# mush42/sonata

Measured on NVIDIA H100. Metric: audio-sec/sec, higher is better.
Workload: dtype f32 io; wgmma with split operands (2 x bf16 flow/decoder, 3 x tf32 encoder/predictor), fp32 accumulate

## Files before the change

### include/sonata_b200.h

```cpp
#ifndef SONATA_B200_H
#define SONATA_B200_H

#include <stddef.h>
#include <stdint.h>

#ifdef __cplusplus
extern "C" {
#endif

#define SB200_OK 0
#define SB200_FAILED_TO_LOAD_RESOURCE 17
#define SB200_PHONEMIZATION_ERROR 18
#define SB200_OPERATION_ERROR 19

typedef struct sb200_voice sb200_voice;
typedef struct sb200_job sb200_job;
typedef struct sb200_latent sb200_latent;

typedef struct sb200_error {
    int32_t code;
    char* message;
} sb200_error;

typedef struct sb200_audio {
// ... 77 lines not shown
int32_t sb200_encode_ids(sb200_voice* v, const int64_t* ids, size_t n, sb200_latent** out, sb200_error* err);
int64_t sb200_latent_frames(const sb200_latent* z);
int32_t sb200_decode_chunk(sb200_voice* v, const sb200_latent* z, int64_t frame_lo, int64_t frame_hi,
                           sb200_audio* out, sb200_error* err);
void sb200_latent_free(sb200_latent* z);

int32_t sb200_encode_batch_ids_configs(sb200_voice* v, const int64_t* ids_packed, const size_t* offsets, size_t batch,
                                       const sb200_synth_config* cfgs, sb200_latent** outs, sb200_error* err);
int32_t sb200_encode_batch_ids_durations(sb200_voice* v, const int64_t* ids_packed, const size_t* offsets, size_t batch,
                                         const sb200_synth_config* cfgs, const float* scale_packed,
                                         const int32_t* frames_packed, sb200_latent** outs, sb200_error* err);
int64_t sb200_latent_id_frames(const sb200_latent* z, int32_t* out, size_t capacity);
int32_t sb200_decode_chunks(sb200_voice* v, const sb200_latent* const* zs, const int64_t* lo, const int64_t* hi, size_t n,
                            sb200_audio* outs, sb200_error* err);
int32_t sb200_decode_chunks_i16(sb200_voice* v, const sb200_latent* const* zs, const int64_t* lo, const int64_t* hi,
                                const int64_t* trim_lo_frames, const int64_t* trim_hi_frames, size_t n, int32_t fade,
                                const float* gain, int16_t** outs, size_t* lens, sb200_error* err);

int32_t sb200_job_debug_fetch(sb200_job* job, const char* name, size_t b, float** data, size_t* rows, size_t* cols,
                              sb200_error* err);
void sb200_buffer_free(float* p);
int32_t sb200_job_debug_durations(sb200_job* job, size_t b, int32_t** cum, size_t* n, sb200_error* err);

typedef struct sb200_region_stat {
    char name[32];
    double ms;
    double flops;
    double bytes;
    int32_t launches;
} sb200_region_stat;
int32_t sb200_job_profile(const sb200_job* job, sb200_region_stat* out, int32_t cap);
int32_t sb200_debug_plan(int32_t backend, int64_t rows, int32_t cin, int32_t cout, int32_t k, int32_t dil, int32_t act,
                         int32_t has_res, int32_t accumulate, int32_t* out16);
int32_t sb200_debug_conv_grid_cap(int32_t cap);
int32_t sb200_debug_conv(int32_t device, int32_t backend, const float* x, int32_t rows, int32_t cin, const float* w,
                         const float* bias, int32_t cout, int32_t k, int32_t dil, float in_slope, int32_t act,
                         const float* res, float scale, int32_t accumulate, float* y, int32_t valid_rows,
                         sb200_error* err);
int32_t sb200_debug_conv_ex(int32_t device, int32_t backend, const float* x, int32_t rows, int32_t cin, const float* w,
                            const float* bias, int32_t cout, int32_t k, int32_t dil, float in_slope, int32_t act,
                            const float* res, float scale, const int32_t* seg_end, int32_t gran, int32_t seg_mul,
                            float* y0, int32_t acc0, int32_t split, float* y1, int32_t acc1, sb200_error* err);
int32_t sb200_debug_spline(int32_t device, const float* h29, int32_t ldh, float* z, int32_t rows, int32_t tcol,
                           int32_t valid_rows, sb200_error* err);
int32_t sb200_debug_durations(int32_t device, const float* z, int32_t rows, const int32_t* seg_off, const int32_t* seg_len,
                              int32_t nseg, float m0, float logs0, float length_scale, float* logw, int32_t* cum,
                              int32_t* y_len, sb200_error* err);
uint64_t sb200_launch_count(void);
int32_t sb200_set_backend(sb200_voice* v, int32_t backend);

#ifdef __cplusplus
}
#endif
#endif
```

### sonata_b200/_native.py

```python
from __future__ import annotations

import ctypes as C
import os

_HERE = os.path.dirname(os.path.abspath(__file__))
LIB_PATH = os.environ.get("SB200_LIB") or os.path.join(_HERE, "lib", "libsonata_b200.so")


class sb200_error(C.Structure):
    _fields_ = [("code", C.c_int32), ("message", C.c_void_p)]


class sb200_audio(C.Structure):
    _fields_ = [("data", C.POINTER(C.c_float)), ("len", C.c_size_t), ("inference_ms", C.c_float),
                ("sample_rate", C.c_uint32)]


class sb200_synth_config(C.Structure):
    _fields_ = [("speaker", C.c_int64), ("has_speaker", C.c_int32), ("noise_scale", C.c_float),
                ("length_scale", C.c_float), ("noise_w", C.c_float)]


class sb200_audio_info(C.Structure):
    _fields_ = [("sample_rate", C.c_uint32), ("num_channels", C.c_uint32), ("sample_width", C.c_uint32)]
# ... 50 lines not shown
    "sb200_job_fetch": (C.c_int32, [_P, C.POINTER(sb200_audio), _ERR]),
    "sb200_job_fetch_i16": (C.c_int32, [_P, C.POINTER(C.POINTER(C.c_int16)), C.POINTER(C.c_size_t), _ERR]),
    "sb200_i16_free": (None, [C.POINTER(C.c_int16)]),
    "sb200_job_batch": (C.c_size_t, [_P]),
    "sb200_job_lengths": (C.c_int32, [_P, C.POINTER(C.c_int64), C.POINTER(C.c_int64), C.POINTER(C.c_int64)]),
    "sb200_job_copy_out": (C.c_int32, [_P, C.c_void_p, C.c_size_t, C.c_int32, C.POINTER(C.c_size_t), _ERR]),
    "sb200_host_register": (C.c_int32, [C.c_void_p, C.c_size_t, _ERR]),
    "sb200_host_unregister": (C.c_int32, [C.c_void_p]),
    "sb200_job_free": (None, [_P]),
    "sb200_encode_ids": (C.c_int32, [_P, C.POINTER(C.c_int64), C.c_size_t, C.POINTER(_P), _ERR]),
    "sb200_latent_frames": (C.c_int64, [_P]),
    "sb200_decode_chunk": (C.c_int32, [_P, _P, C.c_int64, C.c_int64, C.POINTER(sb200_audio), _ERR]),
    "sb200_latent_free": (None, [_P]),
    "sb200_encode_batch_ids_configs": (C.c_int32, [_P, C.POINTER(C.c_int64), C.POINTER(C.c_size_t), C.c_size_t,
                                                   C.POINTER(sb200_synth_config), C.POINTER(_P), _ERR]),
    "sb200_encode_batch_ids_durations": (C.c_int32, [_P, C.POINTER(C.c_int64), C.POINTER(C.c_size_t), C.c_size_t,
                                                     C.POINTER(sb200_synth_config), C.POINTER(C.c_float),
                                                     C.POINTER(C.c_int32), C.POINTER(_P), _ERR]),
    "sb200_latent_id_frames": (C.c_int64, [_P, C.POINTER(C.c_int32), C.c_size_t]),
    "sb200_decode_chunks": (C.c_int32, [_P, C.POINTER(_P), C.POINTER(C.c_int64), C.POINTER(C.c_int64), C.c_size_t,
                                        C.POINTER(sb200_audio), _ERR]),
    "sb200_decode_chunks_i16": (C.c_int32, [_P, C.POINTER(_P), C.POINTER(C.c_int64), C.POINTER(C.c_int64),
                                            C.POINTER(C.c_int64), C.POINTER(C.c_int64), C.c_size_t, C.c_int32,
                                            C.POINTER(C.c_float), C.POINTER(C.POINTER(C.c_int16)),
                                            C.POINTER(C.c_size_t), _ERR]),
    "sb200_job_debug_fetch": (C.c_int32, [_P, C.c_char_p, C.c_size_t, C.POINTER(C.POINTER(C.c_float)),
                                          C.POINTER(C.c_size_t), C.POINTER(C.c_size_t), _ERR]),
    "sb200_buffer_free": (None, [C.POINTER(C.c_float)]),
    "sb200_job_debug_durations": (C.c_int32, [_P, C.c_size_t, C.POINTER(C.POINTER(C.c_int32)),
                                              C.POINTER(C.c_size_t), _ERR]),
    "sb200_job_profile": (C.c_int32, [_P, C.POINTER(sb200_region_stat), C.c_int32]),
    "sb200_debug_plan": (C.c_int32, [C.c_int32, C.c_int64, C.c_int32, C.c_int32, C.c_int32, C.c_int32, C.c_int32, C.c_int32,
                                      C.c_int32, C.POINTER(C.c_int32)]),
    "sb200_debug_conv_grid_cap": (C.c_int32, [C.c_int32]),
    "sb200_debug_conv": (C.c_int32, [C.c_int32, C.c_int32, C.POINTER(C.c_float), C.c_int32, C.c_int32,
                                     C.POINTER(C.c_float), C.POINTER(C.c_float), C.c_int32, C.c_int32, C.c_int32,
                                     C.c_float, C.c_int32, C.POINTER(C.c_float), C.c_float, C.c_int32,
                                     C.POINTER(C.c_float), C.c_int32, _ERR]),
    "sb200_debug_conv_ex": (C.c_int32, [C.c_int32, C.c_int32, C.POINTER(C.c_float), C.c_int32, C.c_int32,
                                        C.POINTER(C.c_float), C.POINTER(C.c_float), C.c_int32, C.c_int32, C.c_int32,
                                        C.c_float, C.c_int32, C.POINTER(C.c_float), C.c_float, C.POINTER(C.c_int32),
                                        C.c_int32, C.c_int32, C.POINTER(C.c_float), C.c_int32, C.c_int32,
                                        C.POINTER(C.c_float), C.c_int32, _ERR]),
    "sb200_debug_spline": (C.c_int32, [C.c_int32, C.POINTER(C.c_float), C.c_int32, C.POINTER(C.c_float), C.c_int32,
                                       C.c_int32, C.c_int32, _ERR]),
    "sb200_debug_durations": (C.c_int32, [C.c_int32, C.POINTER(C.c_float), C.c_int32, C.POINTER(C.c_int32),
                                          C.POINTER(C.c_int32), C.c_int32, C.c_float, C.c_float, C.c_float,
                                          C.POINTER(C.c_float), C.POINTER(C.c_int32), C.POINTER(C.c_int32), _ERR]),
    "sb200_launch_count": (C.c_uint64, []),
    "sb200_set_backend": (C.c_int32, [_P, C.c_int32]),
}

_lib = None


def lib() -> C.CDLL:
    global _lib
    if _lib is None:
        if not os.path.exists(LIB_PATH):
            raise ImportError(
                f"{LIB_PATH} is missing: run `python -c 'import __graft_entry__ as g; g.build()'` "
                "(libsonata_b200 has no CPU fallback)")
        l = C.CDLL(LIB_PATH)
        for name, (res, args) in SIGNATURES.items():
            fn = getattr(l, name)
            fn.restype = res
# ... 4 lines not shown
```

### sonata_b200/csrc/capi.cu

```cuda
#include "../../include/sonata_b200.h"
#include "engine.h"
#include "tc_common.cuh"
#include <algorithm>
#include <chrono>
#include <cstring>
#include <deque>

using namespace sb200;

struct sb200_voice { std::shared_ptr<Voice> v; };
struct sb200_job {
    Job* j; std::shared_ptr<Voice> keep;
    ~sb200_job() { delete j; }
};
struct sb200_latent {
    Latent* l; std::shared_ptr<Voice> keep;
    ~sb200_latent() { delete l; }
};

namespace {

struct PinnedBlock { std::atomic<int> refs{0}; float* base = nullptr; size_t bytes = 0; };
std::mutex g_pin_mu;
std::deque<PinnedBlock*> g_pin_free;
// ... 422 lines not shown
        SB_CUDA(cudaSetDevice(j.v->device));
        if (U < 0) {
            SB_CUDA(cudaMemcpy2D(*data, nr * 4, it->second.first + r0, (size_t)j.RX * 4, nr * 4, (size_t)C, cudaMemcpyDeviceToHost));
            *rows = (size_t)C; *cols = nr;
            return;
        }
        SB_CUDA(cudaMemcpy(*data, it->second.first + r0 * C, nr * C * 4, cudaMemcpyDeviceToHost));
        *rows = nr; *cols = (size_t)C;
    });
}
int32_t sb200_job_debug_durations(sb200_job* job, size_t b, int32_t** cum, size_t* n, sb200_error* err) {
    return guarded(err, [&] {
        Job& j = *job->j;
        if (!j.ran) throw Error(19, "job not run");
        const size_t len = (size_t)j.xsegs[b].len;
        *cum = (int32_t*)malloc(len * 4 + 4);
        SB_CUDA(cudaSetDevice(j.v->device));
        SB_CUDA(cudaMemcpy(*cum, j.d_cum + j.xsegs[b].off, len * 4, cudaMemcpyDeviceToHost));
        *n = len;
    });
}
int32_t sb200_job_profile(const sb200_job* job, sb200_region_stat* out, int32_t cap) {
    const Job& j = *job->j;
    int32_t n = 0;
    for (const Region& r : j.regions) {
        if (n >= cap) break;
        memset(&out[n], 0, sizeof(out[n]));
        strncpy(out[n].name, r.name.c_str(), sizeof(out[n].name) - 1);
        out[n].ms = r.ms; out[n].flops = r.flops; out[n].bytes = r.bytes; out[n].launches = r.launches;
        n++;
    }
    return n;
}
int32_t sb200_debug_plan(int32_t backend, int64_t rows, int32_t cin, int32_t cout, int32_t k, int32_t dil, int32_t act,
                         int32_t has_res, int32_t accumulate, int32_t* out16) {
    if (!out16 || cin <= 0 || cout <= 0 || k <= 0 || k > SB_MAX_TAPS || dil <= 0 || rows <= 0) return 19;
    static float anchor[64];
    float* const stand_in = reinterpret_cast<float*>((reinterpret_cast<uintptr_t>(anchor) + 127) & ~(uintptr_t)127);
    ConvArgs p{};
    const int R = (int)((rows + 255) / 256 * 256);
    const int ycols = act == ACT_GATE ? cout / 2 : cout;
    p.x = stand_in; p.ldx = cin; p.rows_in = R; p.cin = cin; p.in_slope = 0.1f;
    p.w = stand_in; p.bias = stand_in; p.ldw = cout; p.cout = cout;
    p.tc_nt = cout <= 128 ? cout : (cout % 128 == 0 ? 128 : (cout % 96 == 0 ? 96 : 0));
    p.wtc = p.tc_nt ? stand_in : nullptr; p.wtf = stand_in;
    p.ntaps = k;
    for (int t = 0; t < k; t++) p.tap_off[t] = (t - (k - 1) / 2) * dil;
    p.min_off = p.tap_off[0]; p.span = (k - 1) * dil;
    p.rows_q = R; p.orow_mul = 1; p.orow_add = 0;
    p.act = act; p.scale = 1.f; p.res = has_res ? stand_in : nullptr; p.ldres = cout;
    p.y0 = stand_in; p.ldy0 = ycols; p.acc0 = accumulate; p.split = cout; p.y1 = stand_in; p.ldy1 = ycols; p.acc1 = accumulate;
    const bool ok = backend == 2 ? conv_tf_plan_info(p, out16) : conv_tc_plan_info(p, out16);
    return ok ? 0 : 19;
}

int32_t sb200_debug_conv_grid_cap(int32_t cap) {
    const int32_t old = g_conv_tc_grid_cap;
    g_conv_tc_grid_cap = cap > 0 ? cap : 0;
    return old;
}

int32_t sb200_debug_conv_ex(int32_t device, int32_t backend, const float* x, int32_t rows, int32_t cin, const float* w,
                            const float* bias, int32_t cout, int32_t k, int32_t dil, float in_slope, int32_t act,
                            const float* res, float scale, const int32_t* seg_end, int32_t gran, int32_t seg_mul,
                            float* y0, int32_t acc0, int32_t split, float* y1, int32_t acc1, sb200_error* err) {
    return guarded(err, [&] {
        if (rows <= 0 || gran <= 0 || seg_mul <= 0 || !seg_end) throw Error(19, "debug conv: bad row map");
        if (split < 0 || split > cout) split = cout;
        if (split < cout && (act == ACT_GATE || !y1)) throw Error(19, "debug conv: a split output needs y1 and no gate");
        SB_CUDA(cudaSetDevice(device));
        Voice tmp; tmp.device = device;
        ConvW cw = debug_make_conv(tmp, w, bias, cout, cin, k, dil);
        const int R = (rows + 255) / 256 * 256;
        const int ycols = act == ACT_GATE ? cout / 2 : cout;
        const int ld0 = std::min(split, ycols), ld1 = cout - split;
        const int ngran = (R + gran - 1) / gran;
        std::vector<int> ends(ngran, 0);
        for (int g = 0; g < ngran && g * gran < rows; g++) ends[g] = seg_end[g];
        float *dx, *dy0 = nullptr, *dy1 = nullptr, *dres = nullptr; int* dend;
        SB_CUDA(cudaMalloc(&dx, (size_t)R * cin * 4)); SB_CUDA(cudaMemset(dx, 0, (size_t)R * cin * 4));
        SB_CUDA(cudaMemcpy(dx, x, (size_t)rows * cin * 4, cudaMemcpyHostToDevice));
        auto upload_y = [&](float*& d, const float* h, int ld) {
            if (ld <= 0) return;
            SB_CUDA(cudaMalloc(&d, (size_t)R * ld * 4)); SB_CUDA(cudaMemset(d, 0, (size_t)R * ld * 4));
            SB_CUDA(cudaMemcpy(d, h, (size_t)rows * ld * 4, cudaMemcpyHostToDevice));
        };
// ... 101 lines not shown
```

### sonata_b200/csrc/common.cuh

```cuda
#pragma once
#include <cuda_runtime.h>
#include <stdint.h>
#include <stdlib.h>
#include <mutex>

#define SB_MAX_TAPS 16

namespace sb200 {

struct RowMap {
    const int* seg_end;
    int gran;
    int seg_mul;
    int rows;
};

__device__ __forceinline__ bool row_valid(const RowMap& m, int q) {
    if (q < 0 || q >= m.rows) return false;
    return q < m.seg_end[q / m.gran] * m.seg_mul;
}

enum ConvAct { ACT_NONE = 0, ACT_RELU = 1, ACT_GATE = 2 };

struct ConvArgs {
// ... 41 lines not shown
    unsigned long long done = 0;
    template <typename F> void run(F&& f) {
        int dev = 0;
        cudaGetDevice(&dev);
        const unsigned long long bit = 1ull << (dev & 63);
        if (__atomic_load_n(&done, __ATOMIC_ACQUIRE) & bit) return;
        std::lock_guard<std::mutex> g(mu);
        if (done & bit) return;
        f();
        __atomic_fetch_or(&done, bit, __ATOMIC_RELEASE);
    }
};

__device__ __forceinline__ void pdl_wait() { asm volatile("griddepcontrol.wait;" ::: "memory"); }
__device__ __forceinline__ void pdl_trigger() { asm volatile("griddepcontrol.launch_dependents;" ::: "memory"); }

template <typename... KArgs, typename... Args>
inline void launch_pdl(void (*kern)(KArgs...), dim3 grid, dim3 block, size_t smem, cudaStream_t st, Args&&... args) {
    static const int allowed = getenv("SB200_NO_PDL") ? 0 : 1;
    cudaLaunchConfig_t cfg{};
    cfg.gridDim = grid; cfg.blockDim = block; cfg.dynamicSmemBytes = smem; cfg.stream = st;
    cudaLaunchAttribute at[1];
    at[0].id = cudaLaunchAttributeProgrammaticStreamSerialization;
    at[0].val.programmaticStreamSerializationAllowed = allowed;
    cfg.attrs = at; cfg.numAttrs = 1;
    cudaLaunchKernelEx(&cfg, kern, KArgs(args)...);
}

#define SB_ENV_ONCE(name) ([]() -> const char* { static const char* v = getenv(name); return v; }())

void launch_conv_simt(const ConvArgs& a, cudaStream_t st);
int conv_simt_bn_for(int cout);
bool conv_tc_supported(const ConvArgs& a);
bool conv_tc_plan_info(const ConvArgs& a, int* out16);
void launch_conv_tc(const ConvArgs& a, cudaStream_t st);
bool try_launch_conv_tc(const ConvArgs& a, cudaStream_t st);
extern int g_conv_tc_grid_cap;
size_t conv_tc_weight_floats(int cin, int cout, int ntaps, int nt);
void conv_tc_build_weights(const float* wt, int ldw, int cin, int cout, int ntaps, int nt, float* out);
bool conv_tf_supported(const ConvArgs& a);
bool conv_tf_plan_info(const ConvArgs& a, int* out16);
void launch_conv_tf(const ConvArgs& a, cudaStream_t st);
bool try_launch_conv_tf(const ConvArgs& a, cudaStream_t st);
size_t conv_tf_weight_floats(int cin, int cout, int ntaps);
void conv_tf_build_weights(const float* wt, int ldw, int cin, int cout, int ntaps, float* out);
bool gemm_tf_supported(const TfGemm& g);
void launch_gemm_tf(const TfGemm& g, cudaStream_t st);
void throw_launch_error(const char* what);

struct SegInfo { int off; int len; };

void launch_embed(const int* ids_rows, const float* emb, float scale, float* x, int rows, int H, cudaStream_t st);
void launch_ln(const float* x, const float* res1, const float* res2, const float* gamma, const float* beta,
               float* out, int C, int act, RowMap map, cudaStream_t st);
void launch_dw_ln_gelu(const float* x, const float* wdw , const float* bdw, int k, int dil,
                       const float* gamma, const float* beta, float* out, int C, RowMap map, cudaStream_t st);
void launch_attn_softmax(float* S, int Tp, const float* qkv, int ldq, const float* relk, const float* relv, int window,
                         float* orel, int ldo, int H, int heads, int RX, const SegInfo* segs, const int* seg_of_gran,
                         int gran, int max_len, cudaStream_t st);
void launch_attention(const float* qkv, int ldq, const float* relk, const float* relv, int window,
                      float* out, int ldo, int H, int heads, const SegInfo* segs, int nseg, int max_len,
                      cudaStream_t st);
size_t attention_smem_bytes(int max_len, int D);
void launch_flow_pre(const float* z, int zcol, const float* w, const float* b, const float* g, float* h,
                     int C, RowMap map, cudaStream_t st);
void launch_spline(const float* h29, int ldh, float* z, int tcol, int bins, float inv_sqrt_filter,
                   RowMap map, cudaStream_t st);
// ... 24 lines not shown
```

### sonata_b200/csrc/conv_tc.cu

```cuda
#include "tc_common.cuh"
#include <algorithm>
#include <stdlib.h>
#include <string.h>

namespace sb200 {

int g_conv_tc_grid_cap = 0;

int wg_num_sms() {
    static int n = 0;
    if (!n) {
        int dev = 0;
        if (cudaGetDevice(&dev) != cudaSuccess || cudaDeviceGetAttribute(&n, cudaDevAttrMultiProcessorCount, dev) != cudaSuccess)
            cudaGetLastError();
        if (n <= 0) n = 132;
    }
    return n;
}

namespace {

using namespace tcx;

struct TcLaunch {
    int nt;
    int wnt;
    int win;
    int ntiles_m, ntiles_n;
    int grid;
    int resident;
    int pairs;
};

constexpr int TC_CONSUMERS = 256;
constexpr int TC_STAGES = 2;
constexpr int TC_BAR_BYTES = 64;

template <int NT> struct TcRoles {
    static constexpr int ctas = NT == 32 ? 2 : 1;
    static constexpr int producers = NT == 32 ? 128 : 256;
    static constexpr int threads = TC_CONSUMERS + producers;
    static constexpr int launch = (65536 / (threads * ctas)) & ~7;
    static constexpr int producer_regs = NT == 32 ? 40 : 32;
    static constexpr int consumer_regs = ((launch * threads - producer_regs * producers) / TC_CONSUMERS) & ~7;
};

template <int NT>
__global__ void __launch_bounds__(TcRoles<NT>::threads, TcRoles<NT>::ctas) conv_tc_kernel(const ConvArgs a, const TcLaunch L) {
    constexpr int NPROD = TcRoles<NT>::producers;
    pdl_trigger();
    extern __shared__ __align__(1024) uint8_t smem_raw[];
    uint8_t* smem = reinterpret_cast<uint8_t*>((reinterpret_cast<uintptr_t>(smem_raw) + 1023) & ~(uintptr_t)1023);
    const int nkb = a.cin / 32, S = TC_STAGES;
    const uint32_t a_buf = (uint32_t)L.win * 128u;
    const uint32_t w_tap = (uint32_t)NT * 128u;
    const uint32_t w_kb = (uint32_t)a.ntaps * w_tap;
    const uint32_t w_bytes = L.resident ? (uint32_t)nkb * w_kb : (uint32_t)S * w_kb;
    const uint32_t A0 = smem_u32(smem), W0 = A0 + S * a_buf;
    const uint32_t FULL = A0 + S * a_buf + w_bytes;
    const uint32_t EMPTY = FULL + 8u * TC_STAGES;
    const uint32_t WRES = EMPTY + 8u * TC_STAGES;
    const int tid = threadIdx.x;
    const int n_tile = (int)blockIdx.x % L.ntiles_n, m_first = (int)blockIdx.x / L.ntiles_n;
    const int m_step = (int)gridDim.x / L.ntiles_n;
    const int nsteps = (L.ntiles_m - m_first + m_step - 1) / m_step * nkb;

    if (tid == 0) {
        for (int s = 0; s < S; s++) {
            mbar_init(FULL + 8u * s, NPROD + (L.resident ? 0 : 1));
            mbar_init(EMPTY + 8u * s, TC_CONSUMERS);
        }
        mbar_init(WRES, 1);
        asm volatile("fence.mbarrier_init.release.cluster;" ::: "memory");
    }
    __syncthreads();

    if (tid >= TC_CONSUMERS) {
        setmaxnreg_dec<TcRoles<NT>::producer_regs>();
        const int ptid = tid - TC_CONSUMERS;
        const int vf = L.wnt / NT;
        const size_t w_image = (size_t)L.wnt * 128u;
        const uint8_t* wsrc = reinterpret_cast<const uint8_t*>(a.wtc) + (size_t)(n_tile / vf) * nkb * a.ntaps * w_image +
                              (size_t)(n_tile % vf) * w_tap;
        auto issue_w = [&](int kb0, int nkb_, uint32_t dst, uint32_t bar) {
            if (ptid == 0) {
                mbar_expect_tx(bar, (uint32_t)nkb_ * w_kb);
                for (int i = 0; i < nkb_ * a.ntaps; i++)
                    bulk_g2s(dst + i * w_tap, wsrc + (size_t)(kb0 * a.ntaps + i) * w_image, w_tap, bar);
            }
        };
        auto issue_a = [&](int j, int s) {
            const int kb = j % nkb, rbase = (m_first + j / nkb * m_step) * 128 + a.min_off;
            for (int idx = ptid; idx < L.win * 8; idx += NPROD) {
                const int gr = rbase + (idx >> 3);
                const bool ok = gr >= 0 && gr < a.rows_in;
                const float* src = ok ? a.x + (size_t)gr * a.ldx + kb * 32 + (idx & 7) * 4 : a.x;
                cp_async16(A0 + s * a_buf + (uint32_t)idx * 16u, src, ok ? 16u : 0u);
            }
            cp_async_commit();
        };

        if (L.resident) issue_w(0, nkb, W0, WRES);
        else issue_w(0, 1, W0, FULL);
        pdl_wait();

        for (int j = 0; j < nsteps; j++) {
            const int s = j & 1;
            if (j >= S) mbar_wait<false>(EMPTY + 8u * s, (uint32_t)((j / S - 1) & 1));
            if (!L.resident && j > 0) issue_w(j % nkb, 1, W0 + s * w_kb, FULL + 8u * s);
            issue_a(j, s);
            cp_async_wait<0>();
            named_bar_sync(1, NPROD);
            const uint32_t img = A0 + s * a_buf;
            const int npiece = L.win * 4;
            const float slope = a.in_slope;
            for (int base = 0; base < npiece; base += NPROD) {
                const int idx = base + ptid;
                const bool live = idx < npiece;
                const uint32_t odd = (uint32_t)(idx >> 2) & 1u;
                float4 v0 = make_float4(0.f, 0.f, 0.f, 0.f), v1 = v0;
                if (live) {
                    const float4 t0 = lds128(img + (uint32_t)idx * 32u + odd * 16u);
                    const float4 t1 = lds128(img + (uint32_t)idx * 32u + 16u - odd * 16u);
                    v0 = odd ? t1 : t0;
                    v1 = odd ? t0 : t1;
                }
                __syncwarp();
                if (live) {
                    const int r = idx >> 2, cc = idx & 3;
                    float e[8] = {v0.x, v0.y, v0.z, v0.w, v1.x, v1.y, v1.z, v1.w};
                    if (slope != 1.f) {
#pragma unroll
                        for (int i = 0; i < 8; i++) e[i] = fmaxf(e[i], e[i] * slope);
                    }
                    uint4 hi, lo;
                    hi.x = split2(e[0], e[1], lo.x);
                    hi.y = split2(e[2], e[3], lo.y);
                    hi.z = split2(e[4], e[5], lo.z);
                    hi.w = split2(e[6], e[7], lo.w);
                    const uint4 first = odd ? lo : hi, second = odd ? hi : lo;
                    sts128u(sw128(img, r, cc + 4 * (int)odd), first);
                    sts128u(sw128(img, r, cc + 4 - 4 * (int)odd), second);
                }
            }
            mbar_arrive(FULL + 8u * s);
        }
        return;
    }

    setmaxnreg_inc<TcRoles<NT>::consumer_regs>();
    pdl_wait();
    const int warp = tid >> 5, lane = tid & 31;
    const int wg = warp >> 2, g = lane >> 2, c = lane & 3;
    const int r0 = wg * 64 + (warp & 3) * 16 + g;
    float acc[NT / 2];
#pragma unroll
    for (int i = 0; i < NT / 2; i++) acc[i] = 0.f;

    const int n0 = n_tile * NT;
    const bool gate = a.act == ACT_GATE;
    const bool grouped = L.pairs && !gate;
    constexpr int NP = NT / 8, G = NT == 32 ? 4 : 8, NG = 2 * NP / G;
    constexpr bool EARLY = NT > 32;
    bool live[2], valid[2];
    const float* bias[2];
    size_t orow0[2];
    auto load_group = [&](int k0, float2 (&rv)[G], float2 (&dv)[G]) {
#pragma unroll
        for (int i = 0; i < G; i++) {
            const int h = (k0 + i) / NP, nb = n0 + 8 * ((k0 + i) % NP) + 2 * c;
            rv[i] = dv[i] = make_float2(0.f, 0.f);
            if (!live[h] || nb >= a.cout || !valid[h]) continue;
            const bool lo_side = nb < a.split;
            if (a.res) rv[i] = *reinterpret_cast<const float2*>(a.res + orow0[h] * a.ldres + nb);
            if (lo_side ? a.acc0 : a.acc1)
                dv[i] = *reinterpret_cast<const float2*>(lo_side ? a.y0 + orow0[h] * a.ldy0 + nb
                                                                 : a.y1 + orow0[h] * a.ldy1 + (nb - a.split));
        }
    };
    auto store_group = [&](int k0, const float2 (&rv)[G], const float2 (&dv)[G]) {
#pragma unroll
        for (int i = 0; i < G; i++) {
            const int h = (k0 + i) / NP, p = (k0 + i) % NP, nb = n0 + 8 * p + 2 * c;
            if (!live[h] || nb >= a.cout) continue;
            float o[2] = {acc[4 * p + 2 * h], acc[4 * p + 2 * h + 1]};
            if (bias[h]) { o[0] += bias[h][nb]; o[1] += bias[h][nb + 1]; }
            if (a.act == ACT_RELU) { o[0] = fmaxf(o[0], 0.f); o[1] = fmaxf(o[1], 0.f); }
            const bool lo_side = nb < a.split;
            const int accum = lo_side ? a.acc0 : a.acc1;
            if (accum && !valid[h]) continue;
            float2 m = make_float2(0.f, 0.f);
            if (a.res && valid[h]) { m.x = rv[i].x * a.scale; m.y = rv[i].y * a.scale; }
            if (accum && valid[h]) { m.x += dv[i].x; m.y += dv[i].y; }
            *reinterpret_cast<float2*>(lo_side ? a.y0 + orow0[h] * a.ldy0 + nb : a.y1 + orow0[h] * a.ldy1 + (nb - a.split)) =
                valid[h] ? make_float2(fmaf(o[0], a.scale, m.x), fmaf(o[1], a.scale, m.y)) : make_float2(0.f, 0.f);
        }
    };

    for (int j = 0; j < nsteps; j++) {
        const int s = j & 1, kb = j % nkb;
        const int m_tile = m_first + j / nkb * m_step;
        const bool last_kb = kb == nkb - 1;
        float2 rv[2][G], dv[2][G];
        auto first_group = [&]() {
#pragma unroll
            for (int h = 0; h < 2; h++) {
                const int q = m_tile * 128 + r0 + 8 * h;
                live[h] = q < a.rows_q;
                valid[h] = false;
                bias[h] = live[h] ? conv_row(a, q, valid[h]) : nullptr;
                orow0[h] = (size_t)q * a.orow_mul + a.orow_add;
            }
            load_group(0, rv[0], dv[0]);
        };
        if (EARLY && last_kb && grouped) first_group();
        mbar_wait<false>(FULL + 8u * s, (uint32_t)((j >> 1) & 1));
        if (L.resident && j == 0) mbar_wait<false>(WRES, 0);
        const uint32_t img = A0 + s * a_buf;
        const uint32_t wst = L.resident ? W0 + kb * w_kb : W0 + s * w_kb;
        auto load_frag = [&](int t, uint32_t (&ah)[2][4], uint32_t (&al)[2][4]) {
            const int R0 = r0 + a.tap_off[t] - a.min_off, R1 = R0 + 8;
#pragma unroll
            for (int ks = 0; ks < 2; ks++) {
                ah[ks][0] = lds32(sw128(img, R0, 2 * ks) + 4u * c);
                ah[ks][1] = lds32(sw128(img, R1, 2 * ks) + 4u * c);
                ah[ks][2] = lds32(sw128(img, R0, 2 * ks + 1) + 4u * c);
                ah[ks][3] = lds32(sw128(img, R1, 2 * ks + 1) + 4u * c);
                al[ks][0] = lds32(sw128(img, R0, 4 + 2 * ks) + 4u * c);
                al[ks][1] = lds32(sw128(img, R1, 4 + 2 * ks) + 4u * c);
                al[ks][2] = lds32(sw128(img, R0, 5 + 2 * ks) + 4u * c);
                al[ks][3] = lds32(sw128(img, R1, 5 + 2 * ks) + 4u * c);
            }
        };
        auto mma_tap = [&](int t, const uint32_t (&ah)[2][4], const uint32_t (&al)[2][4]) {
            const uint32_t wimg = wst + t * w_tap;
            wg_fence();
#pragma unroll
            for (int ks = 0; ks < 2; ks++) {
                const uint64_t dwh = sw128_desc(wimg + 32u * ks);
                const uint64_t dwl = sw128_desc(wimg + 64u + 32u * ks);
                wgmma_rs<WG_BF16, NT>(acc, ah[ks], dwh);
                wgmma_rs<WG_BF16, NT>(acc, al[ks], dwh);
                wgmma_rs<WG_BF16, NT>(acc, ah[ks], dwl);
            }
            wg_commit();
        };
        uint32_t ah0[2][4], al0[2][4], ah1[2][4], al1[2][4];
        acc_fence<NT / 2>(acc);
        for (int t = 0; t < a.ntaps; t += 2) {
            load_frag(t, ah0, al0);
            mma_tap(t, ah0, al0);
            wg_wait1();
            if (t + 1 < a.ntaps) {
                load_frag(t + 1, ah1, al1);
                mma_tap(t + 1, ah1, al1);
                wg_wait1();
            }
        }
        wg_wait0();
        acc_fence<NT / 2>(acc);
        mbar_arrive(EMPTY + 8u * s);
        if (!last_kb) continue;

        if (grouped) {
            if (!EARLY) first_group();
#pragma unroll
            for (int k = 0; k < NG; k++) {
                const int b = EARLY ? k & 1 : 0;
                if (EARLY && k + 1 < NG) load_group((k + 1) * G, rv[b ^ 1], dv[b ^ 1]);
                if (!EARLY && k > 0) load_group(k * G, rv[0], dv[0]);
                store_group(k * G, rv[b], dv[b]);
            }
        } else {
#pragma unroll
            for (int h = 0; h < 2; h++) {
                const int q = m_tile * 128 + r0 + 8 * h;
                if (q >= a.rows_q) continue;
                bool valid;
                const float* bias = conv_row(a, q, valid);
                const size_t orow0 = (size_t)q * a.orow_mul + a.orow_add;
#pragma unroll
                for (int p = 0; p < NT / 8; p++) {
                    const int nb = n0 + 8 * p + 2 * c;
                    if (nb >= a.cout) continue;
                    float o[2] = {acc[4 * p + 2 * h], acc[4 * p + 2 * h + 1]};
                    if (bias) { o[0] += bias[nb]; o[1] += bias[nb + 1]; }
                    if (gate) {
                        a.y0[orow0 * a.ldy0 + (nb >> 1)] = valid ? tanhf(o[0]) * (1.f / (1.f + expf(-o[1]))) * a.scale : 0.f;
                        continue;
                    }
                    if (a.act == ACT_RELU) { o[0] = fmaxf(o[0], 0.f); o[1] = fmaxf(o[1], 0.f); }
#pragma unroll
                    for (int e = 0; e < 2; e++) {
                        const int n = nb + e;
                        const bool lo_side = n < a.split;
                        const int accum = lo_side ? a.acc0 : a.acc1;
                        if (accum && !valid) continue;
                        float m = 0.f;
                        if (a.res && valid) m = a.res[orow0 * a.ldres + n] * a.scale;
                        float* dst = lo_side ? a.y0 + orow0 * a.ldy0 + n : a.y1 + orow0 * a.ldy1 + (n - a.split);
                        if (accum && valid) m += *dst;
                        *dst = valid ? fmaf(o[e], a.scale, m) : 0.f;
                    }
                }
            }
        }
#pragma unroll
        for (int i = 0; i < NT / 2; i++) acc[i] = 0.f;
    }
}

size_t smem_bytes(const ConvArgs& a, int nt, int win, bool resident) {
    const size_t w_kb = (size_t)a.ntaps * nt * 128;
    return (size_t)TC_STAGES * win * 128 + (resident ? (size_t)(a.cin / 32) : (size_t)TC_STAGES) * w_kb + TC_BAR_BYTES;
}

template <int NT> void allow_smem() {
    static PerDeviceOnce once;
    once.run([] { cudaFuncSetAttribute(conv_tc_kernel<NT>, cudaFuncAttributeMaxDynamicSharedMemorySize, 227 * 1024); });
}

template <int NT> int occupancy(size_t smem) {
    allow_smem<NT>();
    int n = 0;
    if (cudaOccupancyMaxActiveBlocksPerMultiprocessor(&n, conv_tc_kernel<NT>, TcRoles<NT>::threads, smem) != cudaSuccess) {
        cudaGetLastError();
        n = 0;
    }
    return n;
}

int ctas_per_sm(int nt, size_t smem) {
    static int cache[4][256];
    int& slot = cache[nt / 32 - 1][std::min<size_t>(smem >> 10, 255)];
    int n = __atomic_load_n(&slot, __ATOMIC_RELAXED);
    if (n > 0) return n;
    switch (nt) {
        case 32: n = occupancy<32>(smem); break;
        case 64: n = occupancy<64>(smem); break;
        case 96: n = occupancy<96>(smem); break;
        default: n = occupancy<128>(smem); break;
    }
    if (n > 0) {
        __atomic_store_n(&slot, n, __ATOMIC_RELAXED);
        return n;
    }
    const int by_regs = nt == 32 ? TcRoles<32>::ctas : TcRoles<128>::ctas;
    return std::max(1, std::min(by_regs, (int)((228u * 1024u) / (smem + 1024))));
}

bool aligned8(const void* p) { return (reinterpret_cast<uintptr_t>(p) & 7) == 0; }

bool plan(const ConvArgs& a, TcLaunch& L, size_t& smem) {
    if (!a.wtc || a.tc_nt <= 0 || a.tc_nt > 128 || a.tc_nt % 32) return false;
    L.wnt = a.tc_nt;
    L.win = (128 + a.span + 7) & ~7;
    const int mt = (a.rows_q + 127) / 128;
    L.nt = 0;
    for (int nt = a.tc_nt; nt >= 32; nt -= 32)
        if (a.tc_nt % nt == 0 && smem_bytes(a, nt, L.win, false) <= WG_SMEM_BUDGET) { L.nt = nt; break; }
    if (!L.nt) return false;
    if (a.cout % a.tc_nt == 0)
        for (int nt = 32; nt < L.nt; nt += 32)
            if (L.nt % nt == 0 && mt * (a.cout / nt) <= wg_num_sms()) { L.nt = nt; break; }
    L.ntiles_m = mt;
    L.ntiles_n = (a.cout + L.nt - 1) / L.nt;
    L.resident = a.cin / 32 <= TC_STAGES;
    smem = smem_bytes(a, L.nt, L.win, L.resident) + 1024;
    int grid = wg_num_sms() * ctas_per_sm(L.nt, smem);
    if (g_conv_tc_grid_cap > 0) grid = std::min(grid, g_conv_tc_grid_cap);
    L.grid = std::min(std::max(L.ntiles_n, grid / L.ntiles_n * L.ntiles_n), L.ntiles_m * L.ntiles_n);
    L.pairs = a.act != ACT_GATE && a.split % 2 == 0 && aligned8(a.y0) && aligned8(a.y1) &&
              a.ldy0 % 2 == 0 && a.ldy1 % 2 == 0 && (!a.res || (aligned8(a.res) && a.ldres % 2 == 0));
    return true;
}

template <int NT> void launch_nt(const ConvArgs& a, const TcLaunch& L, size_t smem, cudaStream_t st) {
    allow_smem<NT>();
    launch_pdl(conv_tc_kernel<NT>, dim3(L.grid), dim3(TcRoles<NT>::threads), smem, st, a, L);
}

uint16_t bf16_rn_host(float f) {
    uint32_t b; memcpy(&b, &f, 4);
    b += 0x7fffu + ((b >> 16) & 1u);
    return (uint16_t)(b >> 16);
}
float bf16_to_float_host(uint16_t h) {
    uint32_t b = (uint32_t)h << 16; float f; memcpy(&f, &b, 4); return f;
}

}

bool conv_tc_plan_info(const ConvArgs& a, int* out) {
    TcLaunch L{}; size_t smem = 0;
    if (a.cin % 32 || a.cout % 32 || a.ntaps > SB_MAX_TAPS || !plan(a, L, smem)) return false;
    const int v[16] = {L.nt, L.wnt, L.ntiles_m, L.ntiles_n, TC_STAGES, (int)smem, L.win, L.grid, L.resident,
                       ctas_per_sm(L.nt, smem), 0, 0, 0, 0, 0, 0};
    for (int i = 0; i < 16; i++) out[i] = v[i];
    return true;
}

bool conv_tc_supported(const ConvArgs& a) {
    TcLaunch L; size_t smem;
    if (a.cin % 32 || a.cout % 32 || a.ntaps > SB_MAX_TAPS) return false;
    return plan(a, L, smem);
}

void launch_conv_tc(const ConvArgs& a, cudaStream_t st) {
    if (!try_launch_conv_tc(a, st)) launch_conv_simt(a, st);
}

bool try_launch_conv_tc(const ConvArgs& a, cudaStream_t st) {
    if (a.cin % 32 || a.cout % 32 || a.ntaps > SB_MAX_TAPS) return false;
    if ((a.ldx & 3) || (reinterpret_cast<uintptr_t>(a.x) & 15)) return false;
    TcLaunch L; size_t smem;
    if (!plan(a, L, smem)) return false;
    switch (L.nt) {
        case 32: launch_nt<32>(a, L, smem, st); break;
        case 64: launch_nt<64>(a, L, smem, st); break;
        case 96: launch_nt<96>(a, L, smem, st); break;
        default: launch_nt<128>(a, L, smem, st); break;
    }
    g_launch_count++;
    check_launch("conv_tc");
    return true;
}

size_t conv_tc_weight_floats(int cin, int cout, int ntaps, int nt) {
    const int ntiles = (cout + nt - 1) / nt;
    return (size_t)ntiles * (cin / 32) * ntaps * nt * 32;
}
// ... 27 lines not shown
```

### sonata_b200/csrc/tc_common.cuh

```cuda
#pragma once
#include "common.cuh"
#include <cuda_bf16.h>
#include <stdio.h>

namespace sb200 {
namespace tcx {

__device__ __forceinline__ uint32_t smem_u32(const void* p) { return (uint32_t)__cvta_generic_to_shared(p); }

__device__ __forceinline__ uint32_t lds32(uint32_t addr) {
    uint32_t v;
    asm volatile("ld.shared.b32 %0, [%1];" : "=r"(v) : "r"(addr));
    return v;
}
__device__ __forceinline__ float4 lds128(uint32_t addr) {
    float4 v;
    asm volatile("ld.shared.v4.f32 {%0, %1, %2, %3}, [%4];" : "=f"(v.x), "=f"(v.y), "=f"(v.z), "=f"(v.w) : "r"(addr));
    return v;
}
__device__ __forceinline__ void sts128u(uint32_t addr, uint4 v) {
    asm volatile("st.shared.v4.b32 [%0], {%1, %2, %3, %4};" ::"r"(addr), "r"(v.x), "r"(v.y), "r"(v.z), "r"(v.w) : "memory");
}
__device__ __forceinline__ void mbar_init(uint32_t bar, uint32_t count) {
    asm volatile("mbarrier.init.shared::cta.b64 [%0], %1;" ::"r"(bar), "r"(count) : "memory");
}
__device__ __forceinline__ void mbar_expect_tx(uint32_t bar, uint32_t bytes) {
    asm volatile("mbarrier.arrive.expect_tx.shared::cta.b64 _, [%0], %1;" ::"r"(bar), "r"(bytes) : "memory");
}
__device__ __forceinline__ void mbar_arrive(uint32_t bar) {
    asm volatile("mbarrier.arrive.shared::cta.b64 _, [%0];" ::"r"(bar) : "memory");
}
__device__ __forceinline__ void named_bar_sync(int id, int nthreads) {
    asm volatile("bar.sync %0, %1;" ::"r"(id), "r"(nthreads) : "memory");
}
__device__ __forceinline__ bool mbar_try(uint32_t bar, uint32_t parity) {
    uint32_t ok;
    asm volatile(
        "{\n\t.reg .pred p;\n\t"
        "mbarrier.try_wait.parity.shared::cta.b64 p, [%1], %2;\n\t"
        "selp.u32 %0, 1, 0, p;\n\t}"
        : "=r"(ok) : "r"(bar), "r"(parity) : "memory");
    return ok != 0;
}
template <bool kPrint = true> __device__ __forceinline__ void mbar_wait(uint32_t bar, uint32_t parity) {
    unsigned spins = 0;
    unsigned long long t0 = 0;
    while (!mbar_try(bar, parity)) {
        if ((++spins & 1023u) != 0) continue;
        unsigned long long now;
        asm volatile("mov.u64 %0, %globaltimer;" : "=l"(now));
        if (t0 == 0) t0 = now;
        if (now - t0 > 2000000000ull) {
            if (kPrint)
                printf("wgmma conv: mbarrier watchdog (block %d thread %d bar %u parity %u)\n", blockIdx.x, threadIdx.x, bar, parity);
            asm volatile("trap;");
        }
    }
}
__device__ __forceinline__ void bulk_g2s(uint32_t dst, const void* src, uint32_t bytes, uint32_t bar) {
    asm volatile("cp.async.bulk.shared::cluster.global.mbarrier::complete_tx::bytes [%0], [%1], %2, [%3];"
                 ::"r"(dst), "l"(src), "r"(bytes), "r"(bar) : "memory");
}
__device__ __forceinline__ void cp_async16(uint32_t dst, const void* src, uint32_t bytes) {
    asm volatile("cp.async.cg.shared.global [%0], [%1], 16, %2;" ::"r"(dst), "l"(src), "r"(bytes) : "memory");
}
__device__ __forceinline__ void cp_async_commit() { asm volatile("cp.async.commit_group;" ::: "memory"); }
__device__ __forceinline__ void fence_async_smem() { asm volatile("fence.proxy.async.shared::cta;" ::: "memory"); }
template <int N> __device__ __forceinline__ void cp_async_wait() { asm volatile("cp.async.wait_group %0;" ::"n"(N) : "memory"); }
template <int N> __device__ __forceinline__ void setmaxnreg_dec() { asm volatile("setmaxnreg.dec.sync.aligned.u32 %0;" ::"n"(N)); }
template <int N> __device__ __forceinline__ void setmaxnreg_inc() { asm volatile("setmaxnreg.inc.sync.aligned.u32 %0;" ::"n"(N)); }

__device__ __forceinline__ uint32_t sw128(uint32_t img, int row, int chunk) {
    return img + (uint32_t)row * 128u + ((uint32_t)(chunk ^ (row & 7)) << 4);
}
__device__ __forceinline__ uint64_t sw128_desc(uint32_t saddr) {
    return (uint64_t)((saddr & 0x3ffffu) >> 4) | ((uint64_t)1 << 16) | ((uint64_t)(1024 >> 4) << 32) | ((uint64_t)1 << 62);
}

__device__ __forceinline__ void wg_fence() { asm volatile("wgmma.fence.sync.aligned;" ::: "memory"); }
__device__ __forceinline__ void wg_commit() { asm volatile("wgmma.commit_group.sync.aligned;" ::: "memory"); }
__device__ __forceinline__ void wg_wait0() { asm volatile("wgmma.wait_group.sync.aligned 0;" ::: "memory"); }
__device__ __forceinline__ void wg_wait1() { asm volatile("wgmma.wait_group.sync.aligned 1;" ::: "memory"); }
template <int NREG> __device__ __forceinline__ void acc_fence(float* d) {
#pragma unroll
    for (int i = 0; i < NREG; i++) asm volatile("" : "+f"(d[i])::"memory");
}

enum WgKind { WG_BF16 = 0, WG_TF32 = 1 };
template <int KIND, int N> __device__ void wgmma_rs(float* d, const uint32_t* a, uint64_t bdesc);
template <> __device__ __forceinline__ void wgmma_rs<WG_BF16, 32>(float* d, const uint32_t* a, uint64_t bdesc) {
    asm volatile(
        "{\n\t.reg .pred p;\n\tsetp.ne.b32 p, 1, 0;\n\t"
        "wgmma.mma_async.sync.aligned.m64n32k16.f32.bf16.bf16 "
        "{%0,%1,%2,%3,%4,%5,%6,%7,%8,%9,%10,%11,%12,%13,%14,%15}, "
        "{%16,%17,%18,%19}, %20, p, 1, 1, 0;\n\t}"
        : "+f"(d[0]), "+f"(d[1]), "+f"(d[2]), "+f"(d[3]), "+f"(d[4]), "+f"(d[5]), "+f"(d[6]), "+f"(d[7]), "+f"(d[8]), "+f"(d[9]), "+f"(d[10]), "+f"(d[11]), "+f"(d[12]), "+f"(d[13]), "+f"(d[14]), "+f"(d[15])
        : "r"(a[0]), "r"(a[1]), "r"(a[2]), "r"(a[3]), "l"(bdesc));
}
template <> __device__ __forceinline__ void wgmma_rs<WG_BF16, 64>(float* d, const uint32_t* a, uint64_t bdesc) {
// ... 103 lines not shown
```

Baseline: 8762.

## Stage residual and accumulate epilogue operands into shared memory via producer cp.async

Producer warps now prefetch the residual and accumulate-source tiles for the next output tile into swizzled shared-memory staging buffers with cp.async, signalled through new SFULL/SFREE mbarriers. The consumer epilogue then reads them with shared loads instead of global loads. This is meant to take global-memory latency off the epilogue critical path and overlap it with the MMA main loop. Staging is enabled only when it fits the shared-memory budget without lowering CTAs per SM, at the cost of extra shared memory, barrier traffic and more producer work.

```diff
diff --git a/include/sonata_b200.h b/include/sonata_b200.h
--- a/include/sonata_b200.h
+++ b/include/sonata_b200.h
@@ -133,6 +133,8 @@
 int32_t sb200_job_profile(const sb200_job* job, sb200_region_stat* out, int32_t cap);
 int32_t sb200_debug_plan(int32_t backend, int64_t rows, int32_t cin, int32_t cout, int32_t k, int32_t dil, int32_t act,
                          int32_t has_res, int32_t accumulate, int32_t* out16);
+int32_t sb200_debug_plan_staging(int64_t rows, int32_t cin, int32_t cout, int32_t k, int32_t dil, int32_t act,
+                                 int32_t has_res, int32_t accumulate, int32_t* staging_bytes);
 int32_t sb200_debug_conv_grid_cap(int32_t cap);
 int32_t sb200_debug_conv(int32_t device, int32_t backend, const float* x, int32_t rows, int32_t cin, const float* w,
                          const float* bias, int32_t cout, int32_t k, int32_t dil, float in_slope, int32_t act,
diff --git a/sonata_b200/_native.py b/sonata_b200/_native.py
--- a/sonata_b200/_native.py
+++ b/sonata_b200/_native.py
@@ -106,6 +106,8 @@
     "sb200_job_profile": (C.c_int32, [_P, C.POINTER(sb200_region_stat), C.c_int32]),
     "sb200_debug_plan": (C.c_int32, [C.c_int32, C.c_int64, C.c_int32, C.c_int32, C.c_int32, C.c_int32, C.c_int32, C.c_int32,
                                       C.c_int32, C.POINTER(C.c_int32)]),
+    "sb200_debug_plan_staging": (C.c_int32, [C.c_int64, C.c_int32, C.c_int32, C.c_int32, C.c_int32, C.c_int32,
+                                              C.c_int32, C.c_int32, C.POINTER(C.c_int32)]),
     "sb200_debug_conv_grid_cap": (C.c_int32, [C.c_int32]),
     "sb200_debug_conv": (C.c_int32, [C.c_int32, C.c_int32, C.POINTER(C.c_float), C.c_int32, C.c_int32,
                                      C.POINTER(C.c_float), C.POINTER(C.c_float), C.c_int32, C.c_int32, C.c_int32,
diff --git a/sonata_b200/csrc/capi.cu b/sonata_b200/csrc/capi.cu
--- a/sonata_b200/csrc/capi.cu
+++ b/sonata_b200/csrc/capi.cu
@@ -478,8 +478,8 @@
     }
     return n;
 }
-int32_t sb200_debug_plan(int32_t backend, int64_t rows, int32_t cin, int32_t cout, int32_t k, int32_t dil, int32_t act,
-                         int32_t has_res, int32_t accumulate, int32_t* out16) {
+static int32_t debug_plan(int32_t backend, int64_t rows, int32_t cin, int32_t cout, int32_t k, int32_t dil, int32_t act,
+                          int32_t has_res, int32_t accumulate, int32_t* out16, int32_t* staging_bytes) {
     if (!out16 || cin <= 0 || cout <= 0 || k <= 0 || k > SB_MAX_TAPS || dil <= 0 || rows <= 0) return 19;
     static float anchor[64];
     float* const stand_in = reinterpret_cast<float*>((reinterpret_cast<uintptr_t>(anchor) + 127) & ~(uintptr_t)127);
@@ -496,8 +496,18 @@
     p.rows_q = R; p.orow_mul = 1; p.orow_add = 0;
     p.act = act; p.scale = 1.f; p.res = has_res ? stand_in : nullptr; p.ldres = cout;
     p.y0 = stand_in; p.ldy0 = ycols; p.acc0 = accumulate; p.split = cout; p.y1 = stand_in; p.ldy1 = ycols; p.acc1 = accumulate;
-    const bool ok = backend == 2 ? conv_tf_plan_info(p, out16) : conv_tc_plan_info(p, out16);
+    const bool ok = backend == 2 ? conv_tf_plan_info(p, out16) : conv_tc_plan_info(p, out16, staging_bytes);
     return ok ? 0 : 19;
+}
+int32_t sb200_debug_plan(int32_t backend, int64_t rows, int32_t cin, int32_t cout, int32_t k, int32_t dil, int32_t act,
+                         int32_t has_res, int32_t accumulate, int32_t* out16) {
+    return debug_plan(backend, rows, cin, cout, k, dil, act, has_res, accumulate, out16, nullptr);
+}
+int32_t sb200_debug_plan_staging(int64_t rows, int32_t cin, int32_t cout, int32_t k, int32_t dil, int32_t act,
+                                 int32_t has_res, int32_t accumulate, int32_t* staging_bytes) {
+    int32_t out16[16];
+    if (!staging_bytes) return 19;
+    return debug_plan(1, rows, cin, cout, k, dil, act, has_res, accumulate, out16, staging_bytes);
 }
 
 int32_t sb200_debug_conv_grid_cap(int32_t cap) {
diff --git a/sonata_b200/csrc/common.cuh b/sonata_b200/csrc/common.cuh
--- a/sonata_b200/csrc/common.cuh
+++ b/sonata_b200/csrc/common.cuh
@@ -97,7 +97,7 @@
 void launch_conv_simt(const ConvArgs& a, cudaStream_t st);
 int conv_simt_bn_for(int cout);
 bool conv_tc_supported(const ConvArgs& a);
-bool conv_tc_plan_info(const ConvArgs& a, int* out16);
+bool conv_tc_plan_info(const ConvArgs& a, int* out16, int* staging_bytes = nullptr);
 void launch_conv_tc(const ConvArgs& a, cudaStream_t st);
 bool try_launch_conv_tc(const ConvArgs& a, cudaStream_t st);
 extern int g_conv_tc_grid_cap;
diff --git a/sonata_b200/csrc/conv_tc.cu b/sonata_b200/csrc/conv_tc.cu
--- a/sonata_b200/csrc/conv_tc.cu
+++ b/sonata_b200/csrc/conv_tc.cu
@@ -30,11 +30,20 @@
     int grid;
     int resident;
     int pairs;
+    int stage;
 };
 
 constexpr int TC_CONSUMERS = 256;
 constexpr int TC_STAGES = 2;
 constexpr int TC_BAR_BYTES = 64;
+
+__device__ __forceinline__ uint32_t stg_addr(uint32_t base, int row, int col) {
+    return sw128(base + (uint32_t)(col >> 5) * 16384u, row, (col >> 2) & 7) + 4u * (uint32_t)(col & 3);
+}
+__device__ __forceinline__ uint32_t opaque(uint32_t v) {
+    asm volatile("mov.b32 %0, %0;" : "+r"(v));
+    return v;
+}
 
 template <int NT> struct TcRoles {
     static constexpr int ctas = NT == 32 ? 2 : 1;
@@ -50,16 +59,23 @@
     constexpr int NPROD = TcRoles<NT>::producers;
     pdl_trigger();
     extern __shared__ __align__(1024) uint8_t smem_raw[];
-    uint8_t* smem = reinterpret_cast<uint8_t*>((reinterpret_cast<uintptr_t>(smem_raw) + 1023) & ~(uintptr_t)1023);
     const int nkb = a.cin / 32, S = TC_STAGES;
+    const bool acc_any = a.acc0 || a.acc1;
+    const bool stage = NT > 32 && L.stage;
     const uint32_t a_buf = (uint32_t)L.win * 128u;
     const uint32_t w_tap = (uint32_t)NT * 128u;
     const uint32_t w_kb = (uint32_t)a.ntaps * w_tap;
     const uint32_t w_bytes = L.resident ? (uint32_t)nkb * w_kb : (uint32_t)S * w_kb;
-    const uint32_t A0 = smem_u32(smem), W0 = A0 + S * a_buf;
-    const uint32_t FULL = A0 + S * a_buf + w_bytes;
+    const uint32_t stg_op = 128u * NT * 4u;
+    const uint32_t raw = smem_u32(smem_raw), A0 = (raw + 1023u) & ~1023u, W0 = A0 + S * a_buf;
+    const uint32_t SRES = W0 + w_bytes;
+    const uint32_t SACC = SRES + (stage && a.res ? stg_op : 0u);
+    const uint32_t data_end = SACC + (stage && acc_any ? stg_op : 0u);
+    const uint32_t FULL = A0 - raw >= (uint32_t)TC_BAR_BYTES ? raw : data_end;
     const uint32_t EMPTY = FULL + 8u * TC_STAGES;
     const uint32_t WRES = EMPTY + 8u * TC_STAGES;
+    const uint32_t SFULL = WRES + 8u;
+    const uint32_t SFREE = SFULL + 8u;
     const int tid = threadIdx.x;
     const int n_tile = (int)blockIdx.x % L.ntiles_n, m_first = (int)blockIdx.x / L.ntiles_n;
     const int m_step = (int)gridDim.x / L.ntiles_n;
@@ -71,6 +87,8 @@
             mbar_init(EMPTY + 8u * s, TC_CONSUMERS);
         }
         mbar_init(WRES, 1);
+        mbar_init(SFULL, NPROD);
+        mbar_init(SFREE, TC_CONSUMERS);
         asm volatile("fence.mbarrier_init.release.cluster;" ::: "memory");
     }
     __syncthreads();
@@ -99,6 +117,27 @@
             }
             cp_async_commit();
         };
+        constexpr int CPR = NT / 4, RSTEP = NPROD / CPR;
+        auto issue_stage = [&](int t) {
+            if (t > 0) mbar_wait<false>(SFREE, (uint32_t)((t - 1) & 1));
+            const int pt = (int)opaque((uint32_t)ptid);
+            if (pt < RSTEP * CPR) {
+                const int col = 4 * (pt % CPR), nb = n_tile * NT + col;
+                const bool lo_side = nb < a.split;
+                const bool rd_res = a.res && nb < a.cout, rd_acc = (lo_side ? a.acc0 : a.acc1) && nb < a.cout;
+                const float* acc_src = lo_side ? a.y0 + nb : a.y1 + (nb - a.split);
+                const int ld_acc = lo_side ? a.ldy0 : a.ldy1;
+                for (int r = pt / CPR; r < 128; r += RSTEP) {
+                    const int q = (m_first + t * m_step) * 128 + r;
+                    const size_t orow = (size_t)q * a.orow_mul + a.orow_add;
+                    const bool ok_res = rd_res && q < a.rows_q, ok_acc = rd_acc && q < a.rows_q;
+                    if (a.res) cp_async16(stg_addr(SRES, r, col), ok_res ? a.res + nb + orow * a.ldres : a.x, ok_res ? 16u : 0u);
+                    if (acc_any) cp_async16(stg_addr(SACC, r, col), ok_acc ? acc_src + orow * ld_acc : a.x, ok_acc ? 16u : 0u);
+                }
+            }
+            cp_async_commit();
+            cp_async_mbar_arrive(SFULL);
+        };
 
         if (L.resident) issue_w(0, nkb, W0, WRES);
         else issue_w(0, 1, W0, FULL);
@@ -109,7 +148,12 @@
             if (j >= S) mbar_wait<false>(EMPTY + 8u * s, (uint32_t)((j / S - 1) & 1));
             if (!L.resident && j > 0) issue_w(j % nkb, 1, W0 + s * w_kb, FULL + 8u * s);
             issue_a(j, s);
-            cp_async_wait<0>();
+            if (stage && j > 0 && (j - 1) % nkb == 0) {
+                issue_stage((j - 1) / nkb);
+                cp_async_wait<1>();
+            } else {
+                cp_async_wait<0>();
+            }
             named_bar_sync(1, NPROD);
             const uint32_t img = A0 + s * a_buf;
             const int npiece = L.win * 4;
@@ -145,6 +189,8 @@
             }
             mbar_arrive(FULL + 8u * s);
         }
+        if (stage && nkb == 1) issue_stage(nsteps - 1);
+        cp_async_wait<0>();
         return;
     }
 
@@ -162,6 +208,7 @@
     const bool grouped = L.pairs && !gate;
     constexpr int NP = NT / 8, G = NT == 32 ? 4 : 8, NG = 2 * NP / G;
     constexpr bool EARLY = NT > 32;
+    const bool early = EARLY && grouped && !stage;
     bool live[2], valid[2];
     const float* bias[2];
     size_t orow0[2];
@@ -176,6 +223,16 @@
             if (lo_side ? a.acc0 : a.acc1)
                 dv[i] = *reinterpret_cast<const float2*>(lo_side ? a.y0 + orow0[h] * a.ldy0 + nb
                                                                  : a.y1 + orow0[h] * a.ldy1 + (nb - a.split));
+        }
+    };
+    const uint32_t stg_thread = (uint32_t)r0 * 128u + ((uint32_t)((c >> 1) ^ (g & 1)) << 4) + 8u * (uint32_t)(c & 1);
+    auto lds_group = [&](int k0, uint32_t thr, uint32_t gh, float2 (&rv)[G], float2 (&dv)[G]) {
+#pragma unroll
+        for (int i = 0; i < G; i++) {
+            const int h = (k0 + i) / NP, p = (k0 + i) % NP;
+            const uint32_t off = thr + (uint32_t)(p >> 2) * 16384u + (uint32_t)h * 1024u + (((uint32_t)(p & 3) ^ gh) << 5);
+            if (a.res) rv[i] = lds64(SRES + off);
+            if (acc_any) dv[i] = lds64(SACC + off);
         }
     };
     auto store_group = [&](int k0, const float2 (&rv)[G], const float2 (&dv)[G]) {
@@ -202,7 +259,7 @@
         const int m_tile = m_first + j / nkb * m_step;
         const bool last_kb = kb == nkb - 1;
         float2 rv[2][G], dv[2][G];
-        auto first_group = [&]() {
+        auto rows_of_tile = [&]() {
 #pragma unroll
             for (int h = 0; h < 2; h++) {
                 const int q = m_tile * 128 + r0 + 8 * h;
@@ -211,9 +268,11 @@
                 bias[h] = live[h] ? conv_row(a, q, valid[h]) : nullptr;
                 orow0[h] = (size_t)q * a.orow_mul + a.orow_add;
             }
+        };
+        if (early && last_kb) {
+            rows_of_tile();
             load_group(0, rv[0], dv[0]);
-        };
-        if (EARLY && last_kb && grouped) first_group();
+        }
         mbar_wait<false>(FULL + 8u * s, (uint32_t)((j >> 1) & 1));
         if (L.resident && j == 0) mbar_wait<false>(WRES, 0);
         const uint32_t img = A0 + s * a_buf;
@@ -262,8 +321,21 @@
         mbar_arrive(EMPTY + 8u * s);
         if (!last_kb) continue;
 
-        if (grouped) {
-            if (!EARLY) first_group();
+        if (grouped && stage) {
+            rows_of_tile();
+            mbar_wait<false>(SFULL, (uint32_t)((j / nkb) & 1));
+            const uint32_t thr = opaque(stg_thread), gh = opaque((uint32_t)g >> 1);
+#pragma unroll
+            for (int k = 0; k < NG; k++) {
+                lds_group(k * G, thr, gh, rv[0], dv[0]);
+                if (k == NG - 1) mbar_arrive(SFREE);
+                store_group(k * G, rv[0], dv[0]);
+            }
+        } else if (grouped) {
+            if (!EARLY) {
+                rows_of_tile();
+                load_group(0, rv[0], dv[0]);
+            }
 #pragma unroll
             for (int k = 0; k < NG; k++) {
                 const int b = EARLY ? k & 1 : 0;
@@ -310,9 +382,10 @@
     }
 }
 
-size_t smem_bytes(const ConvArgs& a, int nt, int win, bool resident) {
+size_t smem_bytes(const ConvArgs& a, int nt, int win, bool resident, int staged) {
     const size_t w_kb = (size_t)a.ntaps * nt * 128;
-    return (size_t)TC_STAGES * win * 128 + (resident ? (size_t)(a.cin / 32) : (size_t)TC_STAGES) * w_kb + TC_BAR_BYTES;
+    return (size_t)TC_STAGES * win * 128 + (resident ? (size_t)(a.cin / 32) : (size_t)TC_STAGES) * w_kb +
+           (size_t)staged * 128 * nt * 4;
 }
 
 template <int NT> void allow_smem() {
@@ -350,6 +423,15 @@
 }
 
 bool aligned8(const void* p) { return (reinterpret_cast<uintptr_t>(p) & 7) == 0; }
+bool aligned16(const void* p, int ld) { return (reinterpret_cast<uintptr_t>(p) & 15) == 0 && ld % 4 == 0; }
+
+int staged_operands(const ConvArgs& a, const TcLaunch& L) {
+    const bool acc = a.acc0 || a.acc1;
+    if (!L.pairs || (!a.res && !acc) || a.split % 4) return 0;
+    if (a.res && !aligned16(a.res, a.ldres)) return 0;
+    if ((a.acc0 && !aligned16(a.y0, a.ldy0)) || (a.acc1 && !aligned16(a.y1, a.ldy1))) return 0;
+    return (a.res ? 1 : 0) + (acc ? 1 : 0);
+}
 
 bool plan(const ConvArgs& a, TcLaunch& L, size_t& smem) {
     if (!a.wtc || a.tc_nt <= 0 || a.tc_nt > 128 || a.tc_nt % 32) return false;
@@ -358,7 +440,7 @@
     const int mt = (a.rows_q + 127) / 128;
     L.nt = 0;
     for (int nt = a.tc_nt; nt >= 32; nt -= 32)
-        if (a.tc_nt % nt == 0 && smem_bytes(a, nt, L.win, false) <= WG_SMEM_BUDGET) { L.nt = nt; break; }
+        if (a.tc_nt % nt == 0 && smem_bytes(a, nt, L.win, false, 0) <= WG_SMEM_BUDGET) { L.nt = nt; break; }
     if (!L.nt) return false;
     if (a.cout % a.tc_nt == 0)
         for (int nt = 32; nt < L.nt; nt += 32)
@@ -366,12 +448,16 @@
     L.ntiles_m = mt;
     L.ntiles_n = (a.cout + L.nt - 1) / L.nt;
     L.resident = a.cin / 32 <= TC_STAGES;
-    smem = smem_bytes(a, L.nt, L.win, L.resident) + 1024;
+    L.pairs = a.act != ACT_GATE && a.split % 2 == 0 && aligned8(a.y0) && aligned8(a.y1) &&
+              a.ldy0 % 2 == 0 && a.ldy1 % 2 == 0 && (!a.res || (aligned8(a.res) && a.ldres % 2 == 0));
+    smem = smem_bytes(a, L.nt, L.win, L.resident, 0) + 1024;
+    const int nst = staged_operands(a, L);
+    const size_t staged = smem_bytes(a, L.nt, L.win, L.resident, nst) + 1024;
+    L.stage = L.nt > 32 && nst > 0 && staged - 1024 <= WG_SMEM_BUDGET && ctas_per_sm(L.nt, staged) == ctas_per_sm(L.nt, smem);
+    if (L.stage) smem = staged;
     int grid = wg_num_sms() * ctas_per_sm(L.nt, smem);
     if (g_conv_tc_grid_cap > 0) grid = std::min(grid, g_conv_tc_grid_cap);
     L.grid = std::min(std::max(L.ntiles_n, grid / L.ntiles_n * L.ntiles_n), L.ntiles_m * L.ntiles_n);
-    L.pairs = a.act != ACT_GATE && a.split % 2 == 0 && aligned8(a.y0) && aligned8(a.y1) &&
-              a.ldy0 % 2 == 0 && a.ldy1 % 2 == 0 && (!a.res || (aligned8(a.res) && a.ldres % 2 == 0));
     return true;
 }
 
@@ -391,12 +477,13 @@
 
 }
 
-bool conv_tc_plan_info(const ConvArgs& a, int* out) {
+bool conv_tc_plan_info(const ConvArgs& a, int* out, int* staging_bytes) {
     TcLaunch L{}; size_t smem = 0;
     if (a.cin % 32 || a.cout % 32 || a.ntaps > SB_MAX_TAPS || !plan(a, L, smem)) return false;
     const int v[16] = {L.nt, L.wnt, L.ntiles_m, L.ntiles_n, TC_STAGES, (int)smem, L.win, L.grid, L.resident,
                        ctas_per_sm(L.nt, smem), 0, 0, 0, 0, 0, 0};
     for (int i = 0; i < 16; i++) out[i] = v[i];
+    if (staging_bytes) *staging_bytes = L.stage ? staged_operands(a, L) * 128 * L.nt * 4 : 0;
     return true;
 }
 
diff --git a/sonata_b200/csrc/tc_common.cuh b/sonata_b200/csrc/tc_common.cuh
--- a/sonata_b200/csrc/tc_common.cuh
+++ b/sonata_b200/csrc/tc_common.cuh
@@ -16,6 +16,11 @@
 __device__ __forceinline__ float4 lds128(uint32_t addr) {
     float4 v;
     asm volatile("ld.shared.v4.f32 {%0, %1, %2, %3}, [%4];" : "=f"(v.x), "=f"(v.y), "=f"(v.z), "=f"(v.w) : "r"(addr));
+    return v;
+}
+__device__ __forceinline__ float2 lds64(uint32_t addr) {
+    float2 v;
+    asm volatile("ld.shared.v2.f32 {%0, %1}, [%2];" : "=f"(v.x), "=f"(v.y) : "r"(addr));
     return v;
 }
 __device__ __forceinline__ void sts128u(uint32_t addr, uint4 v) {
@@ -65,6 +70,9 @@
     asm volatile("cp.async.cg.shared.global [%0], [%1], 16, %2;" ::"r"(dst), "l"(src), "r"(bytes) : "memory");
 }
 __device__ __forceinline__ void cp_async_commit() { asm volatile("cp.async.commit_group;" ::: "memory"); }
+__device__ __forceinline__ void cp_async_mbar_arrive(uint32_t bar) {
+    asm volatile("cp.async.mbarrier.arrive.noinc.shared::cta.b64 [%0];" ::"r"(bar) : "memory");
+}
 __device__ __forceinline__ void fence_async_smem() { asm volatile("fence.proxy.async.shared::cta;" ::: "memory"); }
 template <int N> __device__ __forceinline__ void cp_async_wait() { asm volatile("cp.async.wait_group %0;" ::"n"(N) : "memory"); }
 template <int N> __device__ __forceinline__ void setmaxnreg_dec() { asm volatile("setmaxnreg.dec.sync.aligned.u32 %0;" ::"n"(N)); }
```

Measured after the change: 9114 (median of 6 runs). 4.0% higher.
